# facebookresearch/vector_db_id_compression

Measured on AMD Instinct MI355X. Metric: IDs encoded+decoded / sec (ROC/ANS, bit-exact vs codec.cpp), higher is better.
Workload: dtype u64

## Files before the change

vector_db_id_compression_amd/csrc/roc_u2.h:

```cpp
#pragma once
#include "roc_u.h"
#include "roc_u2_geom.h"

namespace vidc {
namespace dev {

template <int UB>
__device__ __forceinline__ uint32_t u2_word_of(uint32_t x) {
    using U = U2Geom<UB>;
    return (((x >> U::ESH) ^ (U::NE - 1u)) << U::GSH) | ((x >> 6) & (U::G - 1u));
}

__device__ __forceinline__ uint32_t u2_dec_word_of(uint32_t x) { return x >> 6; }

typedef uint4 U2Div;

template <int UB>
__device__ __forceinline__ void u2_build_counts(const uint64_t *bm, uint32_t &E1, v32u &ra, v32u &rb) {
    using U = U2Geom<UB>;
    const uint32_t lane = lane_id();
    uint32_t running = 0;
    E1 = 0;
#pragma unroll
    for (int L1 = 63; L1 >= 0; L1--) {
// ... 806 lines not shown
    v32u ra, rb;
#pragma unroll
    for (int L1 = 0; L1 < 64; L1++) {
        uint32_t v = 0;
        if ((uint32_t)L1 < NBLK) {
            const uint32_t b0 = 4096u * (NBLK - 1u - (uint32_t)L1);
            const uint32_t in_block = n > b0 ? n - b0 : 0u, want = 64u * (63u - lane);
            v = in_block < want ? in_block : want;
        }
        if (L1 < 32) ra[L1] = v; else rb[L1 - 32] = v;
    }

    const uint32_t p0 = P < 16u ? P : 16u, p1 = P > 16u ? P - 16u : 0u;
    WStack st;
    {
        const uint64_t ao = rfl64(arena_at(a, l));
        ws_init_empty(st, a.arena + ao, rfl((uint32_t)(arena_at(a, l + 1) - ao)), a.mt, VIDC_MT_TABLE);
    }
    uint64_t head = VIDC_RANS_L;
    uint32_t obuf = 0, obase = 0;
    uint32_t *order = WANT_ORDER ? a.perm + off : nullptr;
    const uint32_t T0 = 0x80000000u >> p0, T1 = 0x80000000u >> p1, MULN = 1u << p1;
    const uint32_t l3off = 0u;

    uint32_t nmax = n;
    while (nmax) {
        if (st.sp - st.lo >= 62u) ws_spill32(st);
        if (nmax < 3u || u2_needs_generic(head)) {
            uint32_t idv;
            const uint32_t x = u2r_slow_step<NE>(head, st, nmax, E1, ra, rb, bm, ids, p0, p1, idv);
            if (WANT_ORDER) {
                if (lane == 0) order[obase] = x;
                obase++;
            }
            nmax--;
            continue;
        }
        uint32_t s_x = 0, s_id = 0, s_mul = 0, s_t = 0, s_waddr = NE * 8u, s_D0 = rfl(nmax), s_left = rfl(nmax - 2u);
        uint64_t s_w = 0, s_B = rfl64(head);
        uint64_t z0 = 0, z1 = 0, z2 = 0;
        uint64_t qh = 0;
        uint32_t rr = 0;
        st.sp = rfl(st.sp);
        st.lo = rfl(st.lo);
        st.err = rfl(st.err);
        obase = rfl(obase);
        const uint64_t idbase = rfl64((uint64_t)ids);
#define U2R_ENC_ASM(BODY)                                                                                                 \
        asm volatile(BODY                                                                                                 \
            : "+{v4}"(E1), "+{v5}"(st.win), "+{v6}"(obuf), "+{v[64:95]}"(ra), "+{v[96:127]}"(rb),                          \
              "+{v[46:47]}"(qh), "+{v48}"(rr), "+{s40}"(s_x), "+{s39}"(s_id), "+{s41}"(s_mul), "+{s[58:59]}"(s_B),          \
              "+{s60}"(st.sp), "+{s61}"(st.lo), "+{s65}"(s_waddr), "+{s[66:67]}"(s_w), "+{s69}"(s_t), "+{s85}"(s_D0),        \
              "+{s86}"(s_left), "+{s87}"(obase), "+{s93}"(st.err), "+{v[20:21]}"(z0), "+{v[36:37]}"(z1), "+{v[40:41]}"(z2) \
            : "{v2}"(lane), "{v3}"(l3off), "{s73}"(T0), "{s74}"(T1), "{s75}"(MULN), "{s76}"(p0), "{s77}"(p1),                \
              "{s[88:89]}"(order), "{s[90:91]}"(st.mem), "{s92}"(st.cap), "{s[94:95]}"(dtab), "{s[36:37]}"(idbase)          \
            : "memory", "vcc", "scc", "v7", "v8", "v9", "v10", "v11", "v12", "v13", "v14", "v15", "v16", "v17", "v18", "v19",  \
              "v22", "v23", "v24", "v25", "v26", "v27", "v28", "v29", "v30", "v31", "v32", "v33", "v34", "v35", "v38", "v39",\
              "v42", "v43", "v44", "v45", "v49", "v50", "v51", "v52", "v54", "v55", "v56", "v57", "v58", "v59",                     \
              "s42", "s43", "s44", "s45", "s46", "s47", "s48", "s49", "s50", "s51", "s52", "s53", "s54", "s55", "s56", "s57",\
              "s62", "s63", "s64", "s68", "s70", "s71", "s72", "s78", "s79", "s80", "s81", "s82", "s83", "s84", "s96",       \
              "s97", "s98", "s99")
#define U2R_BODY(XORC)                                                                                                                      \
        if (WANT_ORDER) U2R_ENC_ASM(U2_ENC_ENTRY U2_ENC_TOP_R U2_ENC_MID_G1 U2_ENC_SLICE1_X("6", XORC) U2_ENC_L3_G1 U2_ENC_BOT_R_T(U2_ENC_ORDER, "", "s_cbranch_scc0 7f\n") \
                                    U2_ENC_TOP_R_NL U2_ENC_MID_G1 U2_ENC_SLICE1_X("6", XORC) U2_ENC_L3_G1 U2_ENC_BOT_R(U2_ENC_ORDER, "") "7:\n" U2_ENC_OUTER(U2_ORDER_FLUSH)); \
        else U2R_ENC_ASM(U2_ENC_ENTRY U2_ENC_TOP_R U2_ENC_MID_G1 U2_ENC_SLICE1_X("6", XORC) U2_ENC_L3_G1 U2_ENC_BOT_R_T("", "s_lshr_b64 s[98:99], s[58:59], 31\n", "s_cbranch_scc0 7f\n") \
                         U2_ENC_TOP_R_NL U2_ENC_MID_G1 U2_ENC_SLICE1_X("6", XORC) U2_ENC_L3_G1 U2_ENC_BOT_R("", "s_lshr_b64 s[98:99], s[58:59], 31\n") "7:\n" U2_ENC_OUTER(""))
        if (NEB == 12) { U2R_BODY("0xfff"); } else { U2R_BODY("0x3ff"); }
#undef U2R_BODY
#undef U2R_ENC_ASM
        head = s_B + (uint64_t)((s_id & 0xffffu) * s_mul + (s_id >> 16));
        bm[s_waddr >> 3] = s_w & ~(1ull << (s_x & 63u));
        ws_window(st);
        if (__builtin_expect((head >> 63) != 0ull, 0)) {
            ws_prepare(st);
            ans_u_push(head, st, 0u, 0u);
            ans_u_push(head, st, 0u, 0u);
        }
        nmax = s_D0 - s_t;
    }
    ws_flush(st);
    if (lane == 0) {
        a.heads[l] = head;
        a.prec[l] = P;
        a.nwords[l] = st.sp;
        a.draws[l] = st.draws;
        a.status[l] = st.err ? ((st.err & 1u) ? VIDC_ST_OVERFLOW : VIDC_ST_MT) : VIDC_ST_OK;
    }
}
template <bool WANT_ORDER, int NEB = 12>
__global__ void __launch_bounds__(64) k_roc_encode_r2(RocEncArgs a, const U2Div *__restrict__ dtab) {
    roc_encode_r2_body<WANT_ORDER, NEB>(a, dtab);
}

#ifdef U2_PROF
#define U2PD(i) "s_memtime s[78:79]\n s_waitcnt lgkmcnt(0)\n s_sub_u32 s81, s78, s80\n s_mov_b32 s80, s78\n v_add_u32 v" #i ", s81, v" #i "\n"
#define U2PD_INIT "s_memtime s[78:79]\n s_waitcnt lgkmcnt(0)\n s_mov_b32 s80, s78\n"
#define U2PD_CLOBBERS , "s78", "s79", "s80", "s81"
#else
#define U2PD(i) ""
#define U2PD_INIT ""
#define U2PD_CLOBBERS
#endif
#define U2_DEC_INSTALL \
    "v_mov_b32 v10, v57\n" \
    "s_add_u32 s68, s85, 64\n" \
    "v_add_u32 v58, s68, v2\n" \
    "v_min_u32 v58, 0x40000, v58\n" \
    "v_lshlrev_b32 v58, 4, v58\n" \
    "global_load_dwordx4 v[54:57], v58, s[94:95]\n"
#define U2_DEC_ENTRY \
    "v_add_u32 v58, s85, v2\n" \
    "v_min_u32 v58, 0x40000, v58\n" \
    "v_lshlrev_b32 v58, 4, v58\n" \
    "global_load_dwordx4 v[54:57], v58, s[94:95]\n" \
    "s_waitcnt vmcnt(0)\n" \
    U2_DEC_INSTALL \
    "s_mov_b32 s69, 0\n" \
    "s_mov_b32 s75, s85\n" \
    "s_min_u32 s70, s86, 64\n" U2PD_INIT

#define U2_DEC_TOP "1:\n" U2_DEC_TOP_L("20", "21", "22", "23")
#define U2_DEC_TOP_L(LA, LB, LC, LD)                    \
    U2PD(130) U2PD(131) \
    "s_and_b32 s46, s58, s73\n"                         \
    "s_lshr_b64 s[58:59], s[58:59], s77\n" \
    "s_lshr_b64 s[98:99], s[58:59], 31\n"              \
    "s_cbranch_scc0 " LA "f\n"                          \
    LB ":\n" \
    "s_and_b32 s40, s58, s74\n"                         \
    "s_lshr_b64 s[58:59], s[58:59], s76\n" \
    "s_lshr_b64 s[98:99], s[58:59], 31\n" \
    "s_cbranch_scc0 " LC "f\n" \
    LD ":\n" \
    "s_pack_ll_b32_b16 s40, s40, s46\n"                 U2PD(132)
#define U2_DEC_IDX_G4 \
    "s_lshr_b32 s45, s40, 8\n"                          \
    "v_lshl_add_u32 v28, s45, 5, v3\n" \
    "v_lshlrev_b32_e64 v29, 2, s45\n"                   \
    "ds_read_b64 v[30:31], v28\n" \
    "ds_read_b32 v29, v29\n"                            \
    "s_bfe_u32 s47, s40, 0x20006\n"                     \
    "s_lshr_b32 s65, s40, 5\n"                          U2PD(133)
#define U2_DEC_IDX_G1 \
    "s_lshr_b32 s45, s40, 6\n" \
    "v_lshl_add_u32 v28, s45, 3, v3\n" \
    "v_lshlrev_b32_e64 v29, 2, s45\n" \
    "ds_read_b64 v[30:31], v28\n" \
    "ds_read_b32 v29, v29\n" \
    "s_lshr_b32 s65, s40, 5\n" U2PD(133)
#define U2_DEC_AFTER_RANK \
    "v_writelane_b32 v6, s40, m0\n"                     \
    "v_ashrrev_i32 v58, 31, v58\n" \
    "v_sub_u32 v4, v4, v58\n"                           U2PD(142)
#define U2_DEC_INS_ADDR "v_mad_u32_u24 v26, s65, v8, v9\n"
#define U2_DEC_MID_U \
    "s_lshr_b32 s43, s45, 6\n"                          \
    "s_and_b32 s44, s45, 63\n"                          \
    "s_bfm_b64 s[66:67], s40, 0\n"                      \
    "s_and_b32 m0, s60, 63\n" U2PD(134) \
    "v_readlane_b32 s62, v10, s69\n"                    \
    "v_readlane_b32 s49, v4, s43\n"                     \
    "v_lshl_add_u32 v38, s43, 8, v11\n"                 \
    "v_sub_u32 v39, s44, v2\n" \
    "v_lshrrev_b32 v39, 31, v39\n"                      \
    "v_writelane_b32 v5, s58, m0\n"                     U2PD(135) \
    "s_cmp_ge_u32 s59, s62\n" \
    "s_cselect_b32 s50, s59, s58\n" \
    "s_cselect_b32 s51, 0, s59\n" \
    "s_addc_u32 s60, s60, 0\n" U2PD(136) \
    "s_mul_i32 s52, s50, s75\n"                         \
    "s_mul_hi_u32 s53, s50, s75\n" \
    "s_mul_i32 s68, s51, s75\n" \
    "s_add_u32 s53, s53, s68\n" \
    "s_mov_b32 m0, s69\n" U2PD(137)
#define U2_DEC_RANK_TAIL_U \
    U2_DEC_INS_ADDR \
    "v_lshlrev_b32_e64 v27, s40, 1\n" \
    "v_writelane_b32 v6, s40, m0\n"                     \
    "ds_or_b32 v26, v27\n"                              \
    "ds_add_u32 v38, v39\n"                             U2PD(141)
#define U2_DEC_RANK_U_G4 \
    "s_waitcnt lgkmcnt(0)\n" \
    "v_bcnt_u32_b32 v32, v30, 0\n" \
    "v_bcnt_u32_b32 v32, v31, v32\n"                    \
    "v_and_b32 v33, s66, v30\n" \
    "v_and_b32 v34, s67, v31\n" \
    "v_add_u32_dpp v35, v32, v32 row_shr:1 row_mask:0xf bank_mask:0xf bound_ctrl:0\n" \
    "v_bcnt_u32_b32 v33, v33, s49\n"                    \
    "v_bcnt_u32_b32 v33, v34, v33\n"                    \
    "v_add_u32_dpp v36, v35, v35 row_shr:2 row_mask:0xf bank_mask:0xf bound_ctrl:0\n" \
    "v_sub_u32 v33, v33, v32\n" \
    "v_cmp_lt_u32 vcc, s43, v2\n" \
    "v_add3_u32 v37, v36, v33, v29\n"                   U2PD(139) \
    "v_addc_co_u32 v4, vcc, 0, v4, vcc\n"               \
    "v_readlane_b32 s64, v37, s47\n" U2PD(140) \
    U2_DEC_RANK_TAIL_U
#define U2_DEC_RANK_U_G1 \
    "s_waitcnt lgkmcnt(0)\n" \
    "v_and_b32 v33, s66, v30\n" \
    "v_and_b32 v34, s67, v31\n" \
    "v_bcnt_u32_b32 v33, v33, s49\n" \
    "v_bcnt_u32_b32 v33, v34, v33\n" \
    "v_cmp_lt_u32 vcc, s43, v2\n" \
    "v_add_u32 v37, v29, v33\n" U2PD(139) \
    "v_addc_co_u32 v4, vcc, 0, v4, vcc\n" \
    "v_readfirstlane_b32 s64, v37\n" U2PD(140) \
    U2_DEC_RANK_TAIL_U
#define U2_DEC_IDX_W \
    "s_lshr_b32 s45, s40, 6\n"                          \
    "v_lshlrev_b32_e64 v28, 3, s45\n" \
    "v_lshlrev_b32_e64 v29, 1, s45\n" \
    "ds_read_b64 v[30:31], v28 offset:32768\n"          \
    "ds_read_u16 v29, v29\n"                            \
    "s_lshr_b32 s65, s40, 5\n"                          U2PD(133)
#define U2_DEC_MID_W \
    "s_lshr_b32 s43, s45, 8\n"                          \
    "s_and_b32 s44, s45, 255\n"                         \
    "s_bfm_b64 s[66:67], s40, 0\n"                      \
    "s_and_b32 m0, s60, 63\n" U2PD(134) \
    "v_readlane_b32 s62, v10, s69\n"                    \
    "v_readlane_b32 s49, v4, s43\n"                     \
    "v_lshl_add_u32 v38, s43, 9, v11\n"                 \
    "v_lshl_add_u32 v39, s44, 4, v3\n"                  \
    "v_med3_i32 v39, v39, 0, 63\n" \
    "v_writelane_b32 v5, s58, m0\n"                     \
    "v_lshlrev_b64 v[34:35], v39, s[54:55]\n"           \
    "v_and_b32 v35, 0x7fffffff, v35\n"                  U2PD(135) \
    "s_cmp_ge_u32 s59, s62\n" \
    "s_cselect_b32 s50, s59, s58\n" \
    "s_cselect_b32 s51, 0, s59\n" \
    "s_addc_u32 s60, s60, 0\n" U2PD(136) \
    "s_mul_i32 s52, s50, s75\n"                         \
    "s_mul_hi_u32 s53, s50, s75\n" \
    "s_mul_i32 s68, s51, s75\n" \
    "s_add_u32 s53, s53, s68\n" \
    "s_mov_b32 m0, s69\n" U2PD(137)
#define U2_DEC_RANK_W \
    "s_waitcnt lgkmcnt(0)\n" \
    "v_and_b32 v32, s66, v30\n" \
    "v_and_b32 v33, s67, v31\n" \
    "v_bcnt_u32_b32 v32, v32, s49\n"                    \
    "v_bcnt_u32_b32 v32, v33, v32\n"                    \
    "v_cmp_lt_u32 vcc, s43, v2\n" \
    "v_add_u32 v37, v29, v32\n"                         U2PD(139) \
    "v_addc_co_u32 v4, vcc, 0, v4, vcc\n"               \
    "v_readfirstlane_b32 s64, v37\n" U2PD(140) \
    U2_DEC_INS_ADDR \
    "v_lshlrev_b32 v27, s40, v12\n"                     \
    "v_writelane_b32 v6, s40, m0\n"                     \
    "ds_or_b32 v26, v27\n"                              \
    "ds_add_u64 v38, v[34:35]\n"                        U2PD(141)
#define U2_DEC_BOT_T_U(RLO, RSPAN)                      \
    "s_sub_u32 s68, s60, s61\n"                         \
    "s_add_u32 s68, s68, " RLO "\n" \
    "s_add_u32 s69, s69, 1\n" \
    "s_add_u32 s75, s75, 1\n" \
    "s_add_u32 s58, s52, s64\n"                         \
    "s_addc_u32 s59, s53, 0\n" \
    "s_cmp_gt_u32 s68, " RSPAN "\n" \
    "s_cselect_b32 s71, 0, s70\n" \
    "s_lshr_b64 s[98:99], s[58:59], 31\n"              \
    "s_cselect_b32 s71, s71, 0\n" U2PD(143) \
    "s_cmp_lt_u32 s69, s71\n"
#define U2_DEC_BOT_NR_U \
    "s_add_u32 s69, s69, 1\n" \
    "s_add_u32 s75, s75, 1\n" \
    "s_add_u32 s58, s52, s64\n"                         \
    "s_addc_u32 s59, s53, 0\n" \
    "s_lshr_b64 s[98:99], s[58:59], 31\n"              \
    "s_cselect_b32 s71, s70, 0\n" U2PD(143) \
    "s_cmp_lt_u32 s69, s71\n"
#define U2_DEC_STEP_U(IDX, MID, RANK, LA, LB, LC, LD) U2_DEC_TOP_L(LA, LB, LC, LD) IDX MID RANK U2_DEC_BOT_NR_U "s_cbranch_scc0 2f\n"
#define U2_DEC_LOOP8_U(IDX, MID, RANK) \
    "1:\n" U2_DEC_STEP_U(IDX, MID, RANK, "20", "21", "22", "23") U2_DEC_STEP_U(IDX, MID, RANK, "30", "31", "32", "33") \
    U2_DEC_STEP_U(IDX, MID, RANK, "40", "41", "42", "43") U2_DEC_STEP_U(IDX, MID, RANK, "50", "51", "52", "53") \
    U2_DEC_STEP_U(IDX, MID, RANK, "60", "61", "62", "63") U2_DEC_STEP_U(IDX, MID, RANK, "70", "71", "72", "73") \
    U2_DEC_STEP_U(IDX, MID, RANK, "80", "81", "82", "83") \
    U2_DEC_TOP_L("90", "91", "92", "93") IDX MID RANK U2_DEC_BOT_T_U("-18", "35") "s_cbranch_scc1 1b\n s_branch 2f\n" \
    U2_DEC_SIDE("20", "21", "22", "23") U2_DEC_SIDE("30", "31", "32", "33") U2_DEC_SIDE("40", "41", "42", "43") \
    U2_DEC_SIDE("50", "51", "52", "53") U2_DEC_SIDE("60", "61", "62", "63") U2_DEC_SIDE("70", "71", "72", "73") \
    U2_DEC_SIDE("80", "81", "82", "83") U2_DEC_SIDE("90", "91", "92", "93") "2:\n"
#define U2_DEC_BOT U2_DEC_BOT_CORE "s_cbranch_scc1 1b\n s_branch 2f\n" U2_DEC_SIDE("20", "21", "22", "23") "2:\n"
#define U2_DEC_BOT_CORE U2_DEC_BOT_CORE_T("-2", "59")
#define U2_DEC_BOT_CORE_T(RLO, RSPAN)                   \
    "s_sub_u32 s68, s60, s61\n"                         \
    "s_add_u32 s68, s68, " RLO "\n" \
    "s_add_u32 s69, s69, 1\n" \
    "s_add_u32 s75, s75, 1\n" \
    "s_add_u32 s72, s72, s64\n"                         \
    "s_add_u32 s58, s52, s72\n"                         \
    "s_addc_u32 s59, s53, 0\n" \
    "s_cmp_gt_u32 s68, " RSPAN "\n" \
    "s_cselect_b32 s71, 0, s70\n" \
    "s_lshr_b64 s[98:99], s[58:59], 31\n"              \
    "s_cselect_b32 s71, s71, 0\n" U2PD(143) \
    "s_cmp_lt_u32 s69, s71\n"
#define U2_DEC_BOT_CORE_NR \
    "s_add_u32 s69, s69, 1\n" \
    "s_add_u32 s75, s75, 1\n" \
    "s_add_u32 s72, s72, s64\n"                         \
    "s_add_u32 s58, s52, s72\n"                         \
    "s_addc_u32 s59, s53, 0\n" \
    "s_lshr_b64 s[98:99], s[58:59], 31\n"              \
    "s_cselect_b32 s71, s70, 0\n" U2PD(143) \
    "s_cmp_lt_u32 s69, s71\n"
#define U2_DEC_RING_LO 18u
#define U2_DEC_RING_HI 53u
#define U2_DEC_SIDE(LA, LB, LC, LD) \
    LA ":\n"                                            \
    "s_sub_u32 s60, s60, 1\n" \
    "s_and_b32 s68, s60, 63\n" \
    "s_mov_b32 s59, s58\n" \
    "v_readlane_b32 s58, v5, s68\n" \
    "s_branch " LB "b\n" \
    LC ":\n" \
    "s_sub_u32 s60, s60, 1\n" \
    "s_and_b32 s68, s60, 63\n" \
    "s_mov_b32 s59, s58\n" \
    "v_readlane_b32 s58, v5, s68\n" \
    "s_branch " LD "b\n"
#define U2_DEC_LOOP4(IDX, MID, RANK) \
    "1:\n" U2_DEC_TOP_L("20", "21", "22", "23") IDX MID RANK U2_DEC_BOT_CORE "s_cbranch_scc0 2f\n" \
    U2_DEC_TOP_L("30", "31", "32", "33") IDX MID RANK U2_DEC_BOT_CORE "s_cbranch_scc0 2f\n" \
    U2_DEC_TOP_L("40", "41", "42", "43") IDX MID RANK U2_DEC_BOT_CORE "s_cbranch_scc0 2f\n" \
    U2_DEC_TOP_L("50", "51", "52", "53") IDX MID RANK U2_DEC_BOT_CORE "s_cbranch_scc1 1b\n s_branch 2f\n" \
    U2_DEC_SIDE("20", "21", "22", "23") U2_DEC_SIDE("30", "31", "32", "33") U2_DEC_SIDE("40", "41", "42", "43") \
    U2_DEC_SIDE("50", "51", "52", "53") "2:\n"
#define U2_DEC_STEP_X(IDX, MID, RANK, LA, LB, LC, LD) U2_DEC_TOP_L(LA, LB, LC, LD) IDX MID RANK U2_DEC_BOT_CORE_NR "s_cbranch_scc0 2f\n"
#define U2_DEC_LOOP8(IDX, MID, RANK) \
    "1:\n" U2_DEC_STEP_X(IDX, MID, RANK, "20", "21", "22", "23") U2_DEC_STEP_X(IDX, MID, RANK, "30", "31", "32", "33") \
    U2_DEC_STEP_X(IDX, MID, RANK, "40", "41", "42", "43") U2_DEC_STEP_X(IDX, MID, RANK, "50", "51", "52", "53") \
    U2_DEC_STEP_X(IDX, MID, RANK, "60", "61", "62", "63") U2_DEC_STEP_X(IDX, MID, RANK, "70", "71", "72", "73") \
    U2_DEC_STEP_X(IDX, MID, RANK, "80", "81", "82", "83") \
    U2_DEC_TOP_L("90", "91", "92", "93") IDX MID RANK U2_DEC_BOT_CORE_T("-18", "35") "s_cbranch_scc1 1b\n s_branch 2f\n" \
    U2_DEC_SIDE("20", "21", "22", "23") U2_DEC_SIDE("30", "31", "32", "33") U2_DEC_SIDE("40", "41", "42", "43") \
    U2_DEC_SIDE("50", "51", "52", "53") U2_DEC_SIDE("60", "61", "62", "63") U2_DEC_SIDE("70", "71", "72", "73") \
    U2_DEC_SIDE("80", "81", "82", "83") U2_DEC_SIDE("90", "91", "92", "93") "2:\n"
#define U2_DEC_LOOP2(IDX, MID, RANK) \
    "1:\n" U2_DEC_TOP_L("20", "21", "22", "23") IDX MID RANK U2_DEC_BOT_CORE "s_cbranch_scc0 2f\n" \
    U2_DEC_TOP_L("30", "31", "32", "33") IDX MID RANK U2_DEC_BOT_CORE "s_cbranch_scc1 1b\n s_branch 2f\n" \
    U2_DEC_SIDE("20", "21", "22", "23") U2_DEC_SIDE("30", "31", "32", "33") "2:\n"
#if defined(VIDC_B2_DBG) && (VIDC_B2_DBG & 4)
#define U2_OUT_STORE ""
#else
#define U2_OUT_STORE "global_store_dwordx2 v58, v[6:7], s[88:89]\n"
#endif
#define U2_DEC_FLUSH \
    "v_cmp_gt_u32 vcc, s72, v2\n" \
    "v_sub_u32 v58, s87, v2\n" \
    "v_lshlrev_b32 v58, 3, v58\n" \
    "s_and_saveexec_b64 s[96:97], vcc\n" \
    U2_OUT_STORE \
    "s_mov_b64 exec, s[96:97]\n" \
    "s_sub_u32 s87, s87, s72\n"
#define U2_DEC_OUTER U2_DEC_OUTER_T("-2", "59")
#define U2_DEC_OUTER_T(RLO, RSPAN) \
    "s_lshr_b64 s[98:99], s[58:59], 31\n" \
    "s_cselect_b32 s99, 0, 1\n"                         \
    "s_sub_u32 s68, s60, s61\n" \
    "s_add_u32 s68, s68, " RLO "\n" \
    "s_cmp_gt_u32 s68, " RSPAN "\n" \
    "s_cselect_b32 s99, 1, s99\n"                       \
    "s_cmp_lt_u32 s69, 64\n" \
    "s_cbranch_scc1 5f\n" \
    "s_waitcnt vmcnt(0)\n"                              \
    "s_mov_b32 s72, 64\n" \
    U2_DEC_FLUSH \
    "s_add_u32 s85, s85, 64\n" \
    "s_sub_u32 s86, s86, 64\n" \
    U2_DEC_INSTALL \
    "s_mov_b32 s69, 0\n" \
    "s_min_u32 s70, s86, 64\n" \
    "5:\n" \
    "s_cmp_ge_u32 s69, s70\n" \
    "s_cbranch_scc1 9f\n" \
    "s_cmp_eq_u32 s99, 0\n" \
    "s_cbranch_scc1 1b\n" \
    "9:\n" \
    "s_mov_b32 s72, s69\n" \
    U2_DEC_FLUSH \
    "s_waitcnt vmcnt(0)\n"

template <int UB>
__device__ __forceinline__ uint32_t u2_slow_dec_step(uint64_t &head, WStack &st, uint32_t nmax, uint32_t &E1, uint32_t *rows,
                                                     uint64_t *bm, uint32_t p0, uint32_t p1) {
    using U = U2Geom<UB>;
    const uint32_t lane = lane_id();
    ws_prepare(st);
    const uint32_t x = ans_id_pop(head, st, p0, p1);
    const uint32_t e = x >> U::ESH, w = u2_dec_word_of(x);
    const uint32_t L1 = e >> 6, L2 = e & 63u, g = w & (U::G - 1u), b = x & 63u;
    uint32_t r = rl(E1, L1) + rfl(rows[e]);
    for (uint32_t j = 0; j < g; j++) r += popc64(rfl64(bm[w - g + j]));
    const uint64_t W = rfl64(bm[w]);
    r += popc64(W & ((1ull << b) - 1ull));
    ans_idx_push(head, st, r, nmax, 0x80000000u / nmax);
    E1 += lane > L1 ? 1u : 0u;
    rows[L1 * 64u + lane] += lane > L2 ? 1u : 0u;
    bm[w] = W | (1ull << b);
    wave_sync();
    return x;
}
__device__ __forceinline__ uint32_t u2w_slow_dec_step(uint64_t &head, WStack &st, uint32_t nmax, uint32_t &E1, unsigned char *smem,
                                                      uint32_t p0, uint32_t p1) {
    using D = U2DecWord;
    const uint32_t lane = lane_id();
    ws_prepare(st);
    const uint32_t x = ans_id_pop(head, st, p0, p1);
    const uint32_t L1 = x >> 14, b = x & 63u;
    uint64_t *word = (uint64_t *)(smem + D::word_addr(x));
    const uint64_t W = rfl64(*word);
    const uint32_t r = rl(E1, L1) + rfl((uint32_t) * (const uint16_t *)(smem + D::row_addr(x))) + popc64(W & ((1ull << b) - 1ull));
    ans_idx_push(head, st, r, nmax, 0x80000000u / nmax);
    E1 += lane > L1 ? 1u : 0u;
    *(uint64_t *)(smem + D::add_addr(x, lane)) += D::add_data(x, lane);
    *word = W | (1ull << b);
    wave_sync();
    return x;
}

template <int UB, bool WORD>
__global__ void __launch_bounds__(64) k_roc_decode_u2(RocDecArgs a, const U2Div *__restrict__ dtab) {
    static_assert(!WORD || UB == 20, "word-granular rows are the 20-bit geometry");
    using U = U2Geom<UB>;
    extern __shared__ __align__(16) unsigned char smem[];
    uint32_t *rows = (uint32_t *)smem;
    uint64_t *bm = (uint64_t *)(smem + (WORD ? U2DecWord::BITMAP_OFF : U::DEC_BITMAP_OFF));
    constexpr uint32_t LDS_CLEAR = WORD ? U2DecWord::LDS_BYTES : U::DEC_LDS_BYTES;
    const uint32_t lane = lane_id();
    const uint32_t wi = blockIdx.x;
    if (wi >= a.nwork) return;
    const uint32_t l = rfl(a.worklist[wi]);
    const uint32_t n = rfl((uint32_t)(a.offsets[l + 1] - a.offsets[l]));
    const uint64_t ooff = rfl64(a.out_off ? a.out_off[wi] : a.offsets[l]);
    {
        uint4 *z = (uint4 *)smem;
        for (uint32_t w = lane; w < LDS_CLEAR / 16u; w += 64) z[w] = make_uint4(0, 0, 0, 0);
    }
    const uint32_t P = rfl(a.prec[l]);
    const uint32_t p0 = P < 16u ? P : 16u, p1 = P > 16u ? (P - 16u > 16u ? 16u : P - 16u) : 0u;
    const uint32_t W0 = rfl(a.nwords[l]);
    WStack st;
    ws_init_loaded(st, a.words + rfl64(a.word_off[l]), W0, a.scratch_words + rfl64(a.scratch_off[wi]), roc_dec_stack_cap(n, W0),
                   rfl(a.draws[l]), a.mt, VIDC_MT_TABLE);
    const uint32_t draws0 = st.draws;
    uint64_t head = rfl64(a.heads[l]);
    uint32_t E1 = 0;
    const uint32_t l3off = WORD ? 16u - 64u * lane : U::DEC_BITMAP_OFF + (U::G == 4u ? (lane & 3u) * 8u : 0u);
    const uint32_t ins_mul = WORD ? U2DecWord::ins_mul(lane) : (lane == 0u ? 4u : 0u);
    const uint32_t ins_add = WORD ? U2DecWord::ins_add(lane) : (lane == 0u ? U::DEC_BITMAP_OFF : U::DEC_STRIP_OFF + 4u * lane);
    const uint32_t row_lane = WORD ? 8u * lane : 4u * lane;
    const uint32_t ins_bit = lane == 0u ? 1u : 0u;
    const uint64_t field_ones = rfl64(U2DecWord::FIELD_ONES);
    const uint32_t M1 = (1u << p1) - 1u, M0 = (1u << p0) - 1u;
    uint64_t *out = a.out + ooff;
    wave_sync();
#ifdef U2_PROF
    uint32_t prof[14] = {0, 0, 0, 0, 0, 0, 0, 0, 0, 0, 0, 0, 0, 0};
#endif

#ifdef U2_PROF2
    uint32_t dbg[4] = {0, 0, 0, 0};
#define U2_DBG(k) dbg[k]++
#else
#define U2_DBG(k)
#endif
    uint32_t i = 0;
    constexpr uint32_t RING_LO = U2_DEC_RING_LO, RING_HI = U2_DEC_RING_HI;
    while (i < n) {
        {
            const uint32_t res = st.sp - st.lo;
            if (res > 56u) ws_spill32(st);
            else if (res < 22u && st.lo != 0u) ws_refill32(st);
        }
        if (lt_2p31(head) || st.sp - st.lo < RING_LO || st.sp - st.lo > RING_HI) {
            U2_DBG(0);
            uint32_t x;
            if constexpr (WORD) x = u2w_slow_dec_step(head, st, i + 1u, E1, smem, p0, p1);
            else x = u2_slow_dec_step<UB>(head, st, i + 1u, E1, rows, bm, p0, p1);
            if (lane == 0) out[n - 1u - i] = (uint64_t)x;
            i++;
            continue;
        }
        U2_DBG(1);
        uint32_t s_t = 0, s_N0 = rfl(i + 1u), s_left = rfl(n - i), s_oidx = rfl(n - 1u - i);
        uint64_t s_h = rfl64(head), oring = 0;
        st.sp = rfl(st.sp);
        st.lo = rfl(st.lo);
#define U2_DEC_IN_W "{v12}"(ins_bit), "{s[54:55]}"(field_ones),
#define U2_DEC_ASM(BODY, ...)                                                                                             \
        asm volatile(BODY                                                                                                 \
            : "+{v4}"(E1), "+{v5}"(st.win), "+{v[6:7]}"(oring),                                                           \
              "+{s[58:59]}"(s_h), "+{s60}"(st.sp), "+{s69}"(s_t), "+{s85}"(s_N0), "+{s86}"(s_left), "+{s87}"(s_oidx)        \
              U2P_OPERANDS                                                                                                 \
            : __VA_ARGS__ "{v2}"(lane), "{v3}"(l3off), "{v8}"(ins_mul), "{v9}"(ins_add), "{v11}"(row_lane), "{s61}"(st.lo), \
              "{s73}"(M1), "{s74}"(M0), "{s76}"(p0), "{s77}"(p1), "{s[88:89]}"(out), "{s[94:95]}"(dtab)                     \
            : "memory", "vcc", "scc", "v10", "v26", "v27", "v28", "v29", "v30", "v31", "v32", "v33", "v34", "v35", "v36",     \
              "v37", "v38", "v39", "v54", "v55", "v56", "v57", "v58", "s40", "s43", "s44", "s45", "s46", "s47", "s49", "s50", \
              "s51", "s52", "s53", "s62", "s64", "s65", "s66", "s67", "s68", "s70", "s71", "s72", "s75", "s96", "s97",       \
              "s98", "s99" U2PD_CLOBBERS)
        if constexpr (WORD) U2_DEC_ASM(U2_DEC_ENTRY U2_DEC_LOOP8_U(U2_DEC_IDX_W, U2_DEC_MID_W, U2_DEC_RANK_W) U2_DEC_OUTER_T("-18", "35"), U2_DEC_IN_W);
        else if (U::G == 4u) U2_DEC_ASM(U2_DEC_ENTRY U2_DEC_LOOP8_U(U2_DEC_IDX_G4, U2_DEC_MID_U, U2_DEC_RANK_U_G4) U2_DEC_OUTER_T("-18", "35"));
        else U2_DEC_ASM(U2_DEC_ENTRY U2_DEC_LOOP8_U(U2_DEC_IDX_G1, U2_DEC_MID_U, U2_DEC_RANK_U_G1) U2_DEC_OUTER_T("-18", "35"));
#undef U2_DEC_ASM
#undef U2_DEC_IN_W
        head = s_h;
        ws_window(st);
        if (__builtin_expect(lt_2p31(head), 0)) {
            ws_prepare(st);
            head = (uint64_t)ws_pop(st) | (head << 32);
        }
        i = s_N0 + s_t - 1u;
    }
    uint32_t bits = 0;
    for (uint32_t w = lane; w < U::BITMAP_BYTES / 8u; w += 64) bits += popc64(bm[w]);
#pragma unroll
    for (int o = 32; o > 0; o >>= 1) bits += (uint32_t)__shfl_xor((int)bits, o, 64);
#ifdef U2_PROF2
    if (lane == 0) { a.slots[0] = dbg[0]; a.slots[1] = dbg[1]; a.slots[2] = rfl(bits); a.slots[3] = n; }
#endif
#ifdef U2_PROF
    if (lane == 0)
        for (int q = 0; q < 14; q++) a.slots[q] = prof[q];
#endif
    if (rfl(bits) != n) {
        wave_sync();
        roc_decode_u_body<UB>(a, smem);
        return;
    }
    if (lane == 0) {
        const bool clean = (head == VIDC_RANS_L) && (st.sp == st.draws - draws0);
        a.end_state[l] = clean ? 0u : 1u;
        a.status[l] = st.err ? ((st.err & 1u) ? VIDC_ST_OVERFLOW : VIDC_ST_MT) : VIDC_ST_OK;
    }
}

#ifndef VIDC_B2_DBG
#define VIDC_B2_DBG 0
#endif
#if VIDC_B2_DBG & 1
#define U2B_ROW_LOAD "v_mov_b32 v31, 0\n"
#else
#define U2B_ROW_LOAD "global_load_dword v31, v28, s[82:83]\n"
#endif
#if VIDC_B2_DBG & 2
#define U2B_MEMBER_STORE ""
#else
#define U2B_MEMBER_STORE "global_store_dword v28, v27, s[82:83]\n"
#endif
#define U2B_DEC_IDX \
    "s_lshr_b32 s48, s40, s78\n"                        \
    "v_lshlrev_b32_e64 v26, 1, s48\n" \
    "ds_read_u16 v30, v26\n"                            \
    "v_lshl_add_u32 v28, s48, 8, v3\n"                  \
    U2B_ROW_LOAD \
    "s_xor_b32 s45, s48, 0xfff\n"
#define U2B_DEC_MID_1 \
    "s_lshr_b32 s43, s45, 6\n"                          \
    "s_and_b32 s44, s45, 63\n"                          \
    "s_set_gpr_idx_on s43, gpr_idx(SRC0)\n" \
    "v_mov_b32 v13, v64\n" \
    "s_set_gpr_idx_off\n" \
    "v_lshrrev_b32 v33, s78, v6\n"                      \
    "v_cmp_eq_u32 vcc, s48, v33\n" \
    "v_cmp_gt_u32 s[66:67], s69, v2\n"                  \
    "v_cmp_gt_u32 s[80:81], s40, v6\n"                  \
    "v_readlane_b32 s49, v4, s43\n"                     \
    "v_readlane_b32 s63, v13, s44\n"                    \
    "v_readlane_b32 s62, v10, s69\n"                    \
    "v_subrev_u32 v58, s43, v2\n" \
    "v_subrev_u32 v59, s44, v2\n" \
    "v_ashrrev_i32 v59, 31, v59\n" \
    "v_sub_u32 v13, v13, v59\n"                         \
    "s_and_b64 s[66:67], s[66:67], vcc\n"               \
    "s_bcnt1_i32_b64 s64, s[66:67]\n" \
    "s_and_b64 s[66:67], s[66:67], s[80:81]\n" \
    "s_bcnt1_i32_b64 s46, s[66:67]\n"
#define U2B_DEC_MID_2 \
    "s_and_b32 m0, s60, 63\n"                           \
    "s_cmp_ge_u32 s59, s62\n" \
    "v_writelane_b32 v5, s58, m0\n" \
    "s_cselect_b32 s50, s59, s58\n" \
    "s_cselect_b32 s51, 0, s59\n" \
    "s_addc_u32 s60, s60, 0\n" \
    "s_mul_i32 s52, s50, s75\n"                         \
    "s_mul_hi_u32 s53, s50, s75\n" \
    "s_mul_i32 s68, s51, s75\n" \
    "s_add_u32 s53, s53, s68\n" \
    "s_add_u32 s72, s49, s63\n" \
    "s_set_gpr_idx_on s43, gpr_idx(DST)\n" \
    "v_mov_b32 v64, v13\n" \
    "s_set_gpr_idx_off\n" \
    "s_mov_b32 m0, s69\n"
#define U2B_DEC_MID U2B_DEC_MID_1 U2B_DEC_MID_2
#define U2B_DEC_IDX_MC \
    "s_lshr_b32 s48, s40, s78\n"                        \
    "v_lshlrev_b32_e64 v26, 1, s48\n" \
    "ds_read_u16 v30, v26\n"                            \
    "v_lshl_add_u32 v28, s48, 8, v3\n" \
    "s_xor_b32 s45, s48, 0xfff\n"
#define U2B_DEC_MID_MC U2B_DEC_MID_1 \
    "s_waitcnt lgkmcnt(0)\n" \
    "v_cmp_gt_u32 s[80:81], v30, v2\n"                  \
    "s_mov_b64 exec, s[80:81]\n" \
    U2B_ROW_LOAD \
    "s_mov_b64 exec, -1\n" \
    U2B_DEC_MID_2
#define U2B_DEC_RANK \
    "s_waitcnt vmcnt(0) lgkmcnt(0)\n" \
    U2B_DEC_RANK_TAIL
#define U2B_DEC_RANK_TAIL \
    "v_cmp_gt_u32 s[66:67], s40, v31\n"                 \
    "v_subrev_u32 v33, s64, v30\n"                      \
    "v_min_u32 v32, 63, v30\n"                          \
    "v_cmp_gt_u32 vcc, v33, v2\n"                       \
    "v_mov_b32 v27, s40\n" \
    "v_lshl_add_u32 v28, v32, 2, v28\n"                 \
    "v_max_u32 v29, v29, v30\n" \
    "s_and_b64 vcc, vcc, s[66:67]\n" \
    "v_add_u32 v32, 1, v30\n" \
    "s_bcnt1_i32_b64 s64, vcc\n" \
    "s_add_u32 s64, s64, s46\n"                         \
    "s_mov_b64 exec, 1\n" \
    U2B_MEMBER_STORE \
    "ds_write_b16 v26, v32\n" \
    "s_mov_b64 exec, -1\n" \
    U2_DEC_AFTER_RANK

#define U2B_DEC_PF \
    "s_waitcnt lgkmcnt(0)\n" \
    "v_readfirstlane_b32 s47, v30\n"                    \
    "s_add_u32 s65, s52, s72\n"                         \
    "s_and_b32 s65, s65, s73\n"                         \
    "s_bfm_b32 s68, s90, 0\n" \
    "s_and_b32 s68, s65, s68\n" \
    "s_add_u32 s68, s68, s47\n" \
    "s_lshr_b32 s68, s68, s90\n"                        \
    "s_min_u32 s68, s68, 1\n"                           \
    "s_lshl_b32 s68, s68, 5\n" \
    "s_add_u32 s68, s68, 31\n"                          \
    "s_bfm_b64 s[80:81], s68, 0\n" \
    "s_lshl_b64 s[80:81], s[80:81], 1\n" \
    "s_or_b32 s80, s80, 1\n" \
    "s_and_b64 s[80:81], s[80:81], s[92:93]\n" \
    "s_lshr_b32 s65, s65, s90\n"                        \
    "s_lshl_b32 s65, s65, 8\n" \
    "v_lshl_add_u32 v34, v2, 3, s65\n" \
    "v_and_b32 v34, 0xfffff, v34\n"                     \
    "s_mov_b64 exec, s[80:81]\n" \
    "global_load_dwordx2 v[36:37], v34, s[82:83]\n" \
    "s_mov_b64 exec, -1\n"
#define U2B_DEC_RANK_PF \
    U2B_DEC_PF \
    "s_waitcnt vmcnt(1)\n" \
    U2B_DEC_RANK_TAIL
#define U2L_DEC_IDX \
// ... 196 lines not shown
```

Before: 58.63 million.

## Predicate ANS pops in decode loop and use mbcnt-based rank with prefetched stack word

```diff
diff --git a/vector_db_id_compression_amd/csrc/roc_u2.h b/vector_db_id_compression_amd/csrc/roc_u2.h
--- a/vector_db_id_compression_amd/csrc/roc_u2.h
+++ b/vector_db_id_compression_amd/csrc/roc_u2.h
@@ -982,11 +982,51 @@
     "v_writelane_b32 v6, s40, m0\n"                     \
     "v_ashrrev_i32 v58, 31, v58\n" \
     "v_sub_u32 v4, v4, v58\n"                           U2PD(142)
+#ifndef U2_DEC_STEP
+#define U2_DEC_STEP 3
+#endif
+#define U2_DEC_TOP_P(LA, LB) \
+    U2PD(130) U2PD(131) \
+    "s_lshr_b64 s[98:99], s[58:59], s56\n"             \
+    "s_cbranch_scc0 " LA "f\n" \
+    "s_and_b32 s46, s58, s73\n"                         \
+    "s_bfe_u32 s40, s58, s57\n"                         \
+    "s_lshr_b64 s[58:59], s[58:59], s63\n"              \
+    "s_lshr_b64 s[98:99], s[58:59], 31\n"              \
+    "s_cselect_b32 s59, s59, s58\n"                     \
+    "s_cselect_b32 s58, s58, s41\n" \
+    "s_addc_u32 s60, s60, -1\n"                         \
+    LB ":\n" \
+    "s_pack_ll_b32_b16 s40, s40, s46\n"                 U2PD(132)
+#define U2_DEC_SIDE_P(LA, LB) \
+    LA ":\n"                                            \
+    "s_and_b32 s46, s58, s73\n" \
+    "s_lshr_b64 s[58:59], s[58:59], s77\n" \
+    "s_sub_u32 s60, s60, 1\n" \
+    "s_mov_b32 s59, s58\n" \
+    "s_mov_b32 s58, s41\n" \
+    "s_and_b32 s40, s58, s74\n" \
+    "s_lshr_b64 s[58:59], s[58:59], s76\n" \
+    "s_branch " LB "b\n"
+#if U2_DEC_STEP & 2
+#define U2_DEC_W_IDX "s_sub_u32 s42, s60, 1\n"
+#define U2_DEC_W_LOAD "v_readlane_b32 s41, v5, s42\n"
+#else
+#define U2_DEC_W_IDX ""
+#define U2_DEC_W_LOAD ""
+#endif
+#if U2_DEC_STEP & 1
+#define U2_DEC_BFM ""
+#else
+#define U2_DEC_BFM "s_bfm_b64 s[66:67], s40, 0\n"
+#endif
 #define U2_DEC_INS_ADDR "v_mad_u32_u24 v26, s65, v8, v9\n"
-#define U2_DEC_MID_U \
+#define U2_DEC_MID_U U2_DEC_MID_U_T("s_bfm_b64 s[66:67], s40, 0\n")
+#define U2_DEC_MID_U1 U2_DEC_MID_U_T(U2_DEC_BFM)
+#define U2_DEC_MID_U_T(BFM) \
     "s_lshr_b32 s43, s45, 6\n"                          \
     "s_and_b32 s44, s45, 63\n"                          \
-    "s_bfm_b64 s[66:67], s40, 0\n"                      \
+    BFM \
     "s_and_b32 m0, s60, 63\n" U2PD(134) \
     "v_readlane_b32 s62, v10, s69\n"                    \
     "v_readlane_b32 s49, v4, s43\n"                     \
@@ -998,12 +1038,14 @@
     "s_cselect_b32 s50, s59, s58\n" \
     "s_cselect_b32 s51, 0, s59\n" \
     "s_addc_u32 s60, s60, 0\n" U2PD(136) \
+    U2_DEC_W_IDX \
     "s_mul_i32 s52, s50, s75\n"                         \
     "s_mul_hi_u32 s53, s50, s75\n" \
     "s_mul_i32 s68, s51, s75\n" \
     "s_add_u32 s53, s53, s68\n" \
     "s_mov_b32 m0, s69\n" U2PD(137)
 #define U2_DEC_RANK_TAIL_U \
+    U2_DEC_W_LOAD                                       \
     U2_DEC_INS_ADDR \
     "v_lshlrev_b32_e64 v27, s40, 1\n" \
     "v_writelane_b32 v6, s40, m0\n"                     \
@@ -1025,17 +1067,28 @@
     "v_addc_co_u32 v4, vcc, 0, v4, vcc\n"               \
     "v_readlane_b32 s64, v37, s47\n" U2PD(140) \
     U2_DEC_RANK_TAIL_U
-#define U2_DEC_RANK_U_G1 \
+#if U2_DEC_STEP & 1
+#define U2_DEC_RANK_1W(T) \
     "s_waitcnt lgkmcnt(0)\n" \
-    "v_and_b32 v33, s66, v30\n" \
-    "v_and_b32 v34, s67, v31\n" \
-    "v_bcnt_u32_b32 v33, v33, s49\n" \
-    "v_bcnt_u32_b32 v33, v34, v33\n" \
+    "v_mbcnt_lo_u32_b32 v" T ", v30, s49\n"             \
+    "v_mbcnt_hi_u32_b32 v" T ", v31, v" T "\n" \
     "v_cmp_lt_u32 vcc, s43, v2\n" \
-    "v_add_u32 v37, v29, v33\n" U2PD(139) \
-    "v_addc_co_u32 v4, vcc, 0, v4, vcc\n" \
-    "v_readfirstlane_b32 s64, v37\n" U2PD(140) \
-    U2_DEC_RANK_TAIL_U
+    "v_add_u32 v37, v29, v" T "\n"                      U2PD(139) \
+    "v_addc_co_u32 v4, vcc, 0, v4, vcc\n"               \
+    "v_readlane_b32 s64, v37, s40\n"                   U2PD(140)
+#else
+#define U2_DEC_RANK_1W(T) \
+    "s_waitcnt lgkmcnt(0)\n" \
+    "v_and_b32 v32, s66, v30\n" \
+    "v_and_b32 v33, s67, v31\n" \
+    "v_bcnt_u32_b32 v32, v32, s49\n"                    \
+    "v_bcnt_u32_b32 v32, v33, v32\n"                    \
+    "v_cmp_lt_u32 vcc, s43, v2\n" \
+    "v_add_u32 v37, v29, v32\n"                         U2PD(139) \
+    "v_addc_co_u32 v4, vcc, 0, v4, vcc\n"               \
+    "v_readfirstlane_b32 s64, v37\n" U2PD(140)
+#endif
+#define U2_DEC_RANK_U_G1 U2_DEC_RANK_1W("33") U2_DEC_RANK_TAIL_U
 #define U2_DEC_IDX_W \
     "s_lshr_b32 s45, s40, 6\n"                          \
     "v_lshlrev_b32_e64 v28, 3, s45\n" \
@@ -1046,7 +1099,7 @@
 #define U2_DEC_MID_W \
     "s_lshr_b32 s43, s45, 8\n"                          \
     "s_and_b32 s44, s45, 255\n"                         \
-    "s_bfm_b64 s[66:67], s40, 0\n"                      \
+    U2_DEC_BFM \
     "s_and_b32 m0, s60, 63\n" U2PD(134) \
     "v_readlane_b32 s62, v10, s69\n"                    \
     "v_readlane_b32 s49, v4, s43\n"                     \
@@ -1060,21 +1113,15 @@
     "s_cselect_b32 s50, s59, s58\n" \
     "s_cselect_b32 s51, 0, s59\n" \
     "s_addc_u32 s60, s60, 0\n" U2PD(136) \
+    U2_DEC_W_IDX \
     "s_mul_i32 s52, s50, s75\n"                         \
     "s_mul_hi_u32 s53, s50, s75\n" \
     "s_mul_i32 s68, s51, s75\n" \
     "s_add_u32 s53, s53, s68\n" \
     "s_mov_b32 m0, s69\n" U2PD(137)
 #define U2_DEC_RANK_W \
-    "s_waitcnt lgkmcnt(0)\n" \
-    "v_and_b32 v32, s66, v30\n" \
-    "v_and_b32 v33, s67, v31\n" \
-    "v_bcnt_u32_b32 v32, v32, s49\n"                    \
-    "v_bcnt_u32_b32 v32, v33, v32\n"                    \
-    "v_cmp_lt_u32 vcc, s43, v2\n" \
-    "v_add_u32 v37, v29, v32\n"                         U2PD(139) \
-    "v_addc_co_u32 v4, vcc, 0, v4, vcc\n"               \
-    "v_readfirstlane_b32 s64, v37\n" U2PD(140) \
+    U2_DEC_RANK_1W("32") \
+    U2_DEC_W_LOAD                                       \
     U2_DEC_INS_ADDR \
     "v_lshlrev_b32 v27, s40, v12\n"                     \
     "v_writelane_b32 v6, s40, m0\n"                     \
@@ -1100,16 +1147,27 @@
     "s_lshr_b64 s[98:99], s[58:59], 31\n"              \
     "s_cselect_b32 s71, s70, 0\n" U2PD(143) \
     "s_cmp_lt_u32 s69, s71\n"
-#define U2_DEC_STEP_U(IDX, MID, RANK, LA, LB, LC, LD) U2_DEC_TOP_L(LA, LB, LC, LD) IDX MID RANK U2_DEC_BOT_NR_U "s_cbranch_scc0 2f\n"
+#if U2_DEC_STEP & 2
+#define U2_DEC_TOP_U(LA, LB, LC, LD) U2_DEC_TOP_P(LA, LB)
+#define U2_DEC_SIDE_U(LA, LB, LC, LD) U2_DEC_SIDE_P(LA, LB)
+#define U2_DEC_ENTRY_U U2_DEC_ENTRY U2_DEC_W_IDX U2_DEC_W_LOAD
+#define U2_DEC_OUTER_U(RLO, RSPAN) U2_DEC_OUTER_TR(RLO, RSPAN, U2_DEC_W_IDX U2_DEC_W_LOAD)
+#else
+#define U2_DEC_TOP_U(LA, LB, LC, LD) U2_DEC_TOP_L(LA, LB, LC, LD)
+#define U2_DEC_SIDE_U(LA, LB, LC, LD) U2_DEC_SIDE(LA, LB, LC, LD)
+#define U2_DEC_ENTRY_U U2_DEC_ENTRY
+#define U2_DEC_OUTER_U(RLO, RSPAN) U2_DEC_OUTER_T(RLO, RSPAN)
+#endif
+#define U2_DEC_STEP_U(IDX, MID, RANK, LA, LB, LC, LD) U2_DEC_TOP_U(LA, LB, LC, LD) IDX MID RANK U2_DEC_BOT_NR_U "s_cbranch_scc0 2f\n"
 #define U2_DEC_LOOP8_U(IDX, MID, RANK) \
     "1:\n" U2_DEC_STEP_U(IDX, MID, RANK, "20", "21", "22", "23") U2_DEC_STEP_U(IDX, MID, RANK, "30", "31", "32", "33") \
     U2_DEC_STEP_U(IDX, MID, RANK, "40", "41", "42", "43") U2_DEC_STEP_U(IDX, MID, RANK, "50", "51", "52", "53") \
     U2_DEC_STEP_U(IDX, MID, RANK, "60", "61", "62", "63") U2_DEC_STEP_U(IDX, MID, RANK, "70", "71", "72", "73") \
     U2_DEC_STEP_U(IDX, MID, RANK, "80", "81", "82", "83") \
-    U2_DEC_TOP_L("90", "91", "92", "93") IDX MID RANK U2_DEC_BOT_T_U("-18", "35") "s_cbranch_scc1 1b\n s_branch 2f\n" \
-    U2_DEC_SIDE("20", "21", "22", "23") U2_DEC_SIDE("30", "31", "32", "33") U2_DEC_SIDE("40", "41", "42", "43") \
-    U2_DEC_SIDE("50", "51", "52", "53") U2_DEC_SIDE("60", "61", "62", "63") U2_DEC_SIDE("70", "71", "72", "73") \
-    U2_DEC_SIDE("80", "81", "82", "83") U2_DEC_SIDE("90", "91", "92", "93") "2:\n"
+    U2_DEC_TOP_U("90", "91", "92", "93") IDX MID RANK U2_DEC_BOT_T_U("-18", "35") "s_cbranch_scc1 1b\n s_branch 2f\n" \
+    U2_DEC_SIDE_U("20", "21", "22", "23") U2_DEC_SIDE_U("30", "31", "32", "33") U2_DEC_SIDE_U("40", "41", "42", "43") \
+    U2_DEC_SIDE_U("50", "51", "52", "53") U2_DEC_SIDE_U("60", "61", "62", "63") U2_DEC_SIDE_U("70", "71", "72", "73") \
+    U2_DEC_SIDE_U("80", "81", "82", "83") U2_DEC_SIDE_U("90", "91", "92", "93") "2:\n"
 #define U2_DEC_BOT U2_DEC_BOT_CORE "s_cbranch_scc1 1b\n s_branch 2f\n" U2_DEC_SIDE("20", "21", "22", "23") "2:\n"
 #define U2_DEC_BOT_CORE U2_DEC_BOT_CORE_T("-2", "59")
 #define U2_DEC_BOT_CORE_T(RLO, RSPAN)                   \
@@ -1184,7 +1242,8 @@
     "s_mov_b64 exec, s[96:97]\n" \
     "s_sub_u32 s87, s87, s72\n"
 #define U2_DEC_OUTER U2_DEC_OUTER_T("-2", "59")
-#define U2_DEC_OUTER_T(RLO, RSPAN) \
+#define U2_DEC_OUTER_T(RLO, RSPAN) U2_DEC_OUTER_TR(RLO, RSPAN, "")
+#define U2_DEC_OUTER_TR(RLO, RSPAN, RELOAD)             \
     "s_lshr_b64 s[98:99], s[58:59], 31\n" \
     "s_cselect_b32 s99, 0, 1\n"                         \
     "s_sub_u32 s68, s60, s61\n" \
@@ -1204,6 +1263,7 @@
     "5:\n" \
     "s_cmp_ge_u32 s69, s70\n" \
     "s_cbranch_scc1 9f\n" \
+    RELOAD \
     "s_cmp_eq_u32 s99, 0\n" \
     "s_cbranch_scc1 1b\n" \
     "9:\n" \
@@ -1283,6 +1343,7 @@
     const uint32_t ins_bit = lane == 0u ? 1u : 0u;
     const uint64_t field_ones = rfl64(U2DecWord::FIELD_ONES);
     const uint32_t M1 = (1u << p1) - 1u, M0 = (1u << p0) - 1u;
+    const uint32_t pop_thr = 31u + p1, pop_bfe = (p0 << 16) | p1, pop_sh = p1 + p0;
     uint64_t *out = a.out + ooff;
     wave_sync();
 #ifdef U2_PROF
@@ -1324,14 +1385,15 @@
               "+{s[58:59]}"(s_h), "+{s60}"(st.sp), "+{s69}"(s_t), "+{s85}"(s_N0), "+{s86}"(s_left), "+{s87}"(s_oidx)        \
               U2P_OPERANDS                                                                                                 \
             : __VA_ARGS__ "{v2}"(lane), "{v3}"(l3off), "{v8}"(ins_mul), "{v9}"(ins_add), "{v11}"(row_lane), "{s61}"(st.lo), \
-              "{s73}"(M1), "{s74}"(M0), "{s76}"(p0), "{s77}"(p1), "{s[88:89]}"(out), "{s[94:95]}"(dtab)                     \
+              "{s73}"(M1), "{s74}"(M0), "{s76}"(p0), "{s77}"(p1), "{s[88:89]}"(out), "{s[94:95]}"(dtab),                    \
+              "{s56}"(pop_thr), "{s57}"(pop_bfe), "{s63}"(pop_sh)                                                            \
             : "memory", "vcc", "scc", "v10", "v26", "v27", "v28", "v29", "v30", "v31", "v32", "v33", "v34", "v35", "v36",     \
-              "v37", "v38", "v39", "v54", "v55", "v56", "v57", "v58", "s40", "s43", "s44", "s45", "s46", "s47", "s49", "s50", \
-              "s51", "s52", "s53", "s62", "s64", "s65", "s66", "s67", "s68", "s70", "s71", "s72", "s75", "s96", "s97",       \
-              "s98", "s99" U2PD_CLOBBERS)
-        if constexpr (WORD) U2_DEC_ASM(U2_DEC_ENTRY U2_DEC_LOOP8_U(U2_DEC_IDX_W, U2_DEC_MID_W, U2_DEC_RANK_W) U2_DEC_OUTER_T("-18", "35"), U2_DEC_IN_W);
-        else if (U::G == 4u) U2_DEC_ASM(U2_DEC_ENTRY U2_DEC_LOOP8_U(U2_DEC_IDX_G4, U2_DEC_MID_U, U2_DEC_RANK_U_G4) U2_DEC_OUTER_T("-18", "35"));
-        else U2_DEC_ASM(U2_DEC_ENTRY U2_DEC_LOOP8_U(U2_DEC_IDX_G1, U2_DEC_MID_U, U2_DEC_RANK_U_G1) U2_DEC_OUTER_T("-18", "35"));
+              "v37", "v38", "v39", "v54", "v55", "v56", "v57", "v58", "s40", "s41", "s42", "s43", "s44", "s45", "s46", "s47", \
+              "s49", "s50", "s51", "s52", "s53", "s62", "s64", "s65", "s66", "s67", "s68", "s70", "s71", "s72", "s75", "s96", \
+              "s97", "s98", "s99" U2PD_CLOBBERS)
+        if constexpr (WORD) U2_DEC_ASM(U2_DEC_ENTRY_U U2_DEC_LOOP8_U(U2_DEC_IDX_W, U2_DEC_MID_W, U2_DEC_RANK_W) U2_DEC_OUTER_U("-18", "35"), U2_DEC_IN_W);
+        else if (U::G == 4u) U2_DEC_ASM(U2_DEC_ENTRY_U U2_DEC_LOOP8_U(U2_DEC_IDX_G4, U2_DEC_MID_U, U2_DEC_RANK_U_G4) U2_DEC_OUTER_U("-18", "35"));
+        else U2_DEC_ASM(U2_DEC_ENTRY_U U2_DEC_LOOP8_U(U2_DEC_IDX_G1, U2_DEC_MID_U1, U2_DEC_RANK_U_G1) U2_DEC_OUTER_U("-18", "35"));
 #undef U2_DEC_ASM
 #undef U2_DEC_IN_W
         head = s_h;
diff --git a/vector_db_id_compression_amd/csrc/u2_pops_ref.h b/vector_db_id_compression_amd/csrc/u2_pops_ref.h
--- /dev/null
+++ b/vector_db_id_compression_amd/csrc/u2_pops_ref.h
@@ -0,0 +1,69 @@
+#pragma once
+#include <stdint.h>
+
+namespace vidc {
+
+enum U2PopClass : uint32_t { U2_POP_NONE = 0, U2_POP_SLICE0 = 1, U2_POP_SLICE1 = 2, U2_POP_BOTH = 3 };
+
+struct U2Pops {
+    uint64_t head;
+    uint32_t x;
+    uint32_t popped;
+    uint32_t cls;
+};
+
+inline uint32_t u2_pop_p1(uint32_t P) { return P > 16u ? (P - 16u > 16u ? 16u : P - 16u) : 0u; }
+inline uint32_t u2_pop_p0(uint32_t P) { return P < 16u ? P : 16u; }
+
+template <class Pop>
+inline U2Pops u2_pops_two(uint64_t head, uint32_t p1, uint32_t p0, Pop pop) {
+    U2Pops r{0, 0, 0, U2_POP_NONE};
+    const uint32_t x_hi = (uint32_t)(head & ((1ull << p1) - 1ull));
+    head >>= p1;
+    if (head < (1ull << 31)) { head = (head << 32) | (uint64_t)pop(); r.popped++; r.cls |= U2_POP_SLICE1; }
+    const uint32_t x_lo = (uint32_t)(head & ((1ull << p0) - 1ull));
+    head >>= p0;
+    if (head < (1ull << 31)) { head = (head << 32) | (uint64_t)pop(); r.popped++; r.cls |= U2_POP_SLICE0; }
+    r.head = head;
+    r.x = (x_hi << 16) | x_lo;
+    return r;
+}
+
+inline uint32_t u2_s_bfe_u32(uint32_t v, uint32_t operand) {
+    const uint32_t off = operand & 31u, width = (operand >> 16) & 127u;
+    if (width == 0u) return 0u;
+    return width >= 32u ? v >> off : (v >> off) & ((1u << width) - 1u);
+}
+
+inline U2Pops u2_pops_one(uint64_t head, uint32_t w, uint32_t p1, uint32_t p0) {
+    const uint32_t thr = 31u + p1, bfe = (p0 << 16) | p1, sh = p1 + p0;
+    const uint32_t m1 = (1u << p1) - 1u, m0 = p0 >= 32u ? ~0u : (1u << p0) - 1u;
+    uint32_t lo = (uint32_t)head, hi = (uint32_t)(head >> 32);
+    U2Pops r{0, 0, 0, U2_POP_NONE};
+    uint32_t x_hi, x_lo;
+    if ((head >> (thr & 63u)) != 0ull) {
+        x_hi = lo & m1;
+        x_lo = u2_s_bfe_u32(lo, bfe);
+        head >>= (sh & 63u);
+        lo = (uint32_t)head; hi = (uint32_t)(head >> 32);
+        const bool scc = (head >> 31) != 0ull;
+        hi = scc ? hi : lo;
+        lo = scc ? lo : w;
+        if (!scc) { r.popped = 1; r.cls = U2_POP_SLICE0; }
+        head = ((uint64_t)hi << 32) | lo;
+    } else {
+        x_hi = lo & m1;
+        head >>= p1;
+        lo = (uint32_t)head;
+        r.popped = 1; r.cls = U2_POP_SLICE1;
+        hi = lo;
+        lo = w;
+        x_lo = lo & m0;
+        head = (((uint64_t)hi << 32) | lo) >> p0;
+    }
+    r.head = head;
+    r.x = ((x_hi & 0xffffu) << 16) | (x_lo & 0xffffu);
+    return r;
+}
+
+}
```

After: 61.44 million (median of 6 runs). 4.8% higher.
